# norlab-ulaval/norlab_icp_mapper

Hardware: AMD Instinct MI355X
Metric: ICP iterations/sec, 100k-pt scan vs 1M-pt map (higher is better)
Workload: dtype f32; 1 GPU; single synthetic 100000-pt scan vs 1000000-pt map, point-to-point ICP, KDTreeMatcher knn 1 maxDist 2.0 epsilon 0, TrimmedDist 0.85, fixed 20 iterations per registration; chain=p2p, scene=box+pillars sigma=0.01 seeds 42/43/44 (SURVEY.md 8d), parallelism=scan-sharded x1, map replicated

## Files before the change

norlab_icp_mapper_amd/csrc/common.h:

```cpp
#pragma once

#include <hip/hip_runtime.h>
#include <stdint.h>
#include <math.h>
#include <cstring>
#include <string>
#include <vector>
#include <unordered_map>
#include <mutex>
#include <map>
#include <cstdlib>
#include <shared_mutex>

#include "../../include/icpmi.h"

#define ICPMI_NV 32
#define ICPMI_MAX_OUTLIER 8
#define ICPMI_MAX_SMOOTH 16
#define ICPMI_SEL_BINS 2048
#ifndef ICPMI_S2_COPIES
#define ICPMI_S2_COPIES 8
#endif
#define ICPMI_S2_C0 4096
#define ICPMI_S2_F0 (ICPMI_S2_C0 + ICPMI_S2_COPIES * 256)
#ifndef ICPMI_S2_FCOPIES
#define ICPMI_S2_FCOPIES 1
#endif
#define ICPMI_S2_C1 (ICPMI_S2_F0 + ICPMI_S2_FCOPIES * 65536)
#define ICPMI_S2_F1 (ICPMI_S2_C1 + 256)
#define ICPMI_ACC_COPIES 2
#define ICPMI_ACC_MAX_ADDS 128
#define ICPMI_ACC_PAD 16
#define ICPMI_ACC_U64 (ICPMI_ACC_COPIES * ICPMI_NV * 2 * ICPMI_ACC_PAD)
#define ICPMI_ACC_IDX(copy, i, limb) ((((copy) * ICPMI_NV + (i)) * 2 + (limb)) * ICPMI_ACC_PAD)
#define ICPMI_ACC_FLAG (ICPMI_ACC_IDX(0, 0, 0) + 8)
#define ICPMI_S2_ACC (ICPMI_S2_F1 + 65536)
#define ICPMI_WIN_BINS 7
#ifndef ICPMI_WIN_COPIES
#define ICPMI_WIN_COPIES 8
#endif
#define ICPMI_WIN_PAD 16
#define ICPMI_WIN_HDR (ICPMI_WIN_COPIES * 3 * ICPMI_WIN_PAD)
#define ICPMI_WIN_U64 (ICPMI_WIN_HDR + ICPMI_WIN_PAD)
#define ICPMI_WIN_MAX_COUNT (1ll << 21)
#define ICPMI_S2_WIN (ICPMI_S2_ACC + 2 * ICPMI_ACC_U64)
#define ICPMI_SELHIST_WORDS (ICPMI_S2_WIN + 2 * ICPMI_WIN_U64)
#define ICPMI_S2_FIDX(b) ((((b) & 255u) << 8) | ((b) >> 8))

#define ICPMI_MAX_K 32

#ifdef __HIPCC__
typedef float icpmi_vf4 __attribute__((ext_vector_type(4)));
#ifdef ICPMI_NT_STREAMS
__device__ __forceinline__ float4 ld_stream(const float4* p) { const icpmi_vf4 v = __builtin_nontemporal_load(reinterpret_cast<const icpmi_vf4*>(p)); return make_float4(v.x, v.y, v.z, v.w); }
__device__ __forceinline__ float ld_stream(const float* p) { return __builtin_nontemporal_load(p); }
__device__ __forceinline__ int ld_stream(const int* p) { return __builtin_nontemporal_load(p); }
// ... 32 lines not shown
    float cell, inv_cell;
    float slack;
    int   nx, ny, nz;
    int   ncells;
};

#define ICPMI_MAXLEV 8
struct GridLevels {
    int nlev;
    GridParams g[ICPMI_MAXLEV];
    const float4* pts[ICPMI_MAXLEV];
    const unsigned* cs[ICPMI_MAXLEV];
    const unsigned* pos0[ICPMI_MAXLEV];
};

#define ICPMI_MAX_BATCH 16
struct BatchArgs {
    int nscan;
    int qstride;
    int n[ICPMI_MAX_BATCH];
};
struct BatchSrc { const float4* p[ICPMI_MAX_BATCH]; };
static inline float squared_radius(float r) { return std::isinf(r) ? INFINITY : r * r; }
static inline BatchArgs batch_of_one(int64_t n) { BatchArgs b; memset(&b, 0, sizeof b); b.nscan = 1; b.n[0] = (int)n; return b; }

struct LoopCfg {
    int   k;
    float max_dist;
    float maxr2;
    float inv1e, err2;
    int   ring_max;
    int   minimizer;
    int   n_out;
    int   out_type[ICPMI_MAX_OUTLIER];
    float out_param[ICPMI_MAX_OUTLIER];
    int   out_iparam[ICPMI_MAX_OUTLIER];
    float out_param2[ICPMI_MAX_OUTLIER];
    float out_param3[ICPMI_MAX_OUTLIER];
    int   ext;
    int   force_4dof;
    int   force_2d;
    int   is_2d;
    int   max_iter;
    int   use_diff;
    float min_rot, min_trans;
    int   smooth;
    int   use_bound;
    float max_rot, max_trans;
    int   has_read_normals;
    int   sensor_noise;
    const float* read_scalar;
};

struct IcpState {
    float T_iter[16];
    int   iter;
    int   done;
    int   error;
    int   stop_reason;
    int   counter;
    int   hist_n;
    double hq[(ICPMI_MAX_SMOOTH + 1) * 4];
    double ht[(ICPMI_MAX_SMOOTH + 1) * 3];
    double hrot[ICPMI_MAX_SMOOTH + 1];
    double htr[ICPMI_MAX_SMOOTH + 1];
    double init_q[4];
    unsigned sel_prefix;
    unsigned sel_rank;
    unsigned n_valid;
    unsigned sel_prefix_l[3];
    unsigned sel_rank_l[3];
    float limits[ICPMI_MAX_OUTLIER];
    unsigned vt_valid;
    float vt_ratio;
    float robust_med;
    float robust_scale;
    long long pairs;
    double wsum;
    unsigned hard_count;
    unsigned ticket;
    unsigned long long hard_total;
    unsigned seq;
    unsigned long long dbg[24];
    float T_prev[16];
    float T_out[16];
    unsigned long long t_start, t_done;
    unsigned long long t_nn_begin, t_nn_sum;
    unsigned nn_count, pad_nn;
};

#ifdef __HIPCC__
__device__ __forceinline__ void nn_stamp_open(IcpState* st) { st->t_nn_begin = (unsigned long long)wall_clock64(); }
__device__ __forceinline__ void nn_stamp_close(IcpState* st)
{
    const unsigned long long b = st->t_nn_begin;
    if (b) { st->t_nn_sum += (unsigned long long)wall_clock64() - b; ++st->nn_count; st->t_nn_begin = 0; }
}
#endif


inline std::shared_mutex& capture_gate() { static std::shared_mutex* m = new std::shared_mutex; return *m; }
struct CaptureGate {
    CaptureGate() { capture_gate().lock_shared(); }
    ~CaptureGate() { capture_gate().unlock_shared(); }
    CaptureGate(const CaptureGate&) = delete;
    CaptureGate& operator=(const CaptureGate&) = delete;
};

struct LoopGraph {
    hipGraphExec_t exec = nullptr; uint64_t sig = 0; int uses = 0; bool sorted = false;
    int len = 0; unsigned long used = 0;
    bool holds(uint64_t s) const { return exec && sig == s; }
    void reset() { if (exec) hipGraphExecDestroy(exec); *this = LoopGraph(); }
};
struct LoopGraphs {
    LoopGraph fixed, batch, seg[2], heads[4];
    unsigned long clock = 0;
    void reset() { fixed.reset(); batch.reset(); for (LoopGraph& g : seg) g.reset(); for (LoopGraph& g : heads) g.reset(); }
};

struct DevBlockCache {
    struct Live { size_t bytes; int dev; };
    std::mutex mu;
    std::unordered_map<void*, Live> live;
    std::map<int, std::multimap<size_t, void*>> idle_of;
    size_t idle_bytes = 0, limit = 0;
    long handles = 0;
    bool on = true;
    DevBlockCache()
    {
        const char* e = getenv("ICPMI_ALLOC_CACHE_MB");
        const long mb = e ? atol(e) : 1024;
        on = mb > 0; limit = on ? (size_t)mb << 20 : 0;
    }
};
inline DevBlockCache& dev_block_cache() { static DevBlockCache* c = new DevBlockCache; return *c; }

inline void dev_cache_release_locked(DevBlockCache& bc)
{
    for (auto& dv : bc.idle_of) for (auto& kv : dv.second) (void)hipFree(kv.second);
    bc.idle_of.clear(); bc.idle_bytes = 0;
}
inline void dev_cache_trim()
{
    DevBlockCache& bc = dev_block_cache();
    std::lock_guard<std::mutex> lk(bc.mu);
    dev_cache_release_locked(bc);
}

inline hipError_t dev_malloc(void** p, size_t bytes)
// ... 720 lines not shown
```

norlab_icp_mapper_amd/csrc/loop.hip:

```cpp
#include "common.h"
#include "solve.h"
#include <cstring>
#include <vector>

namespace {

template <int PASS, int MODE = 0>
__global__ __launch_bounds__(256) void sel_hist_kernel(const float* __restrict__ d2, int64_t count,
                                                       const IcpState* __restrict__ st, unsigned* __restrict__ ghist, int nb_scale = 0)
{
    if (st->done) return;
    if (blockIdx.x == 0 && threadIdx.x == 0) nn_stamp_close(const_cast<IcpState*>(st));
    if (MODE != 0 && nb_scale != 0 && st->iter + 1 > nb_scale) return;
    if (MODE == 3 && st->iter != 0) return;
    __shared__ unsigned h[ICPMI_SEL_BINS];
    for (int b = threadIdx.x; b < ICPMI_SEL_BINS; b += 256) h[b] = 0;
    __syncthreads();
    const unsigned prefix = st->sel_prefix;
    const float med = MODE == 2 ? st->robust_med : 0.f;
    for (int64_t i = (int64_t)blockIdx.x * 256 + threadIdx.x; i < count; i += (int64_t)gridDim.x * 256) {
        float v = d2[i];
        if (MODE == 0 || MODE == 3) { if (!(v != INFINITY && v > 0.f)) continue; }
        else {
            if (v == INFINITY) continue;
// ... 230 lines not shown
        if (win_lookup(hists, quantile, shw, pf, rr, tot)) return;
    }
#ifndef ICPMI_H0_PF
#define ICPMI_H0_PF 16
#endif
    constexpr int PF = ICPMI_H0_PF;
    const int64_t stride = (int64_t)gridDim.x * 256;
    const int64_t i0 = (int64_t)blockIdx.x * 256 + threadIdx.x;
    float pv[PF];
#pragma unroll
    for (int u = 0; u < PF; ++u) pv[u] = i0 + u * stride < count ? d2[i0 + u * stride] : INFINITY;
    if (st->done) return;
    constexpr int WIN = 4096;
    __shared__ unsigned h[256];
    __shared__ unsigned win[WIN];
    __shared__ unsigned s_top;
    h[threadIdx.x] = 0;
    for (int i = threadIdx.x; i < WIN; i += 256) win[i] = 0;
    if (threadIdx.x == 0) s_top = 0u;
    for (int64_t i = i0; i < 256 + 65536; i += stride) hists[ICPMI_S2_C1 + i] = 0;
    __syncthreads();
    {
        unsigned mx = 0;
#pragma unroll
        for (int u = 0; u < PF; ++u) if (pv[u] != INFINITY && pv[u] > 0.f) mx = max(mx, __float_as_uint(pv[u]) >> 16);
        for (int off = 32; off > 0; off >>= 1) mx = max(mx, (unsigned)__shfl_xor((int)mx, off, 64));
        if ((threadIdx.x & 63) == 0 && mx) atomicMax(&s_top, mx);
    }
    __syncthreads();
    const unsigned top = s_top + 1u, lo = top > (unsigned)WIN ? top - (unsigned)WIN : 0u;
    unsigned* fine = hists + ICPMI_S2_F0 + (blockIdx.x % ICPMI_S2_FCOPIES) * 65536;
    auto add = [&](float v) {
        if (!(v != INFINITY && v > 0.f)) return;
        const unsigned bits = __float_as_uint(v);
        const unsigned bin = bits >> 16, rel = bin - lo;
        if (rel < (unsigned)WIN) atomicAdd(&win[rel], 1u);
        else { atomicAdd(&h[bits >> 24], 1u); atomicAdd(&fine[ICPMI_S2_FIDX(bin)], 1u); }
    };
#pragma unroll
    for (int u = 0; u < PF; ++u) add(pv[u]);
    for (int64_t i = i0 + PF * stride; i < count; i += stride) add(d2[i]);
    __syncthreads();
    for (int i = threadIdx.x; i < WIN; i += 256) {
        const unsigned cnt = win[i];
        if (cnt) { const unsigned bin = lo + (unsigned)i; atomicAdd(&h[bin >> 8], cnt); atomicAdd(&fine[ICPMI_S2_FIDX(bin)], cnt); }
    }
    __syncthreads();
    if (h[threadIdx.x]) atomicAdd(&hists[ICPMI_S2_C0 + (blockIdx.x % ICPMI_S2_COPIES) * 256 + threadIdx.x], h[threadIdx.x]);
}

__global__ __launch_bounds__(256) void sel2_scan_hist_kernel(const float* __restrict__ d2, BatchArgs ba, int k, IcpState* __restrict__ st,
                                                             unsigned* __restrict__ hists, float quantile, int use_win)
{
    const int64_t count = (int64_t)ba.n[blockIdx.y] * k;
    d2 += (size_t)blockIdx.y * (size_t)ba.qstride * k;
    hists += (size_t)blockIdx.y * ICPMI_SELHIST_WORDS;
    st += blockIdx.y;
    constexpr int PF = 2;
    const int64_t stride = (int64_t)gridDim.x * 256;
    const int64_t i0 = (int64_t)blockIdx.x * 256 + threadIdx.x;
    float pv[PF];
#pragma unroll
    for (int u = 0; u < PF; ++u) pv[u] = i0 + u * stride < count ? d2[i0 + u * stride] : INFINITY;
    unsigned cv = 0;
#pragma unroll
    for (int cpy = 0; cpy < ICPMI_S2_COPIES; ++cpy) cv += hists[ICPMI_S2_C0 + cpy * 256 + threadIdx.x];
    if (st->done) return;
    if (blockIdx.x == 0 && threadIdx.x == 0) nn_stamp_close(const_cast<IcpState*>(st));
    __shared__ unsigned sh[16];
    unsigned prefix, rem, total;
    const bool win_hit = use_win && win_lookup(hists, quantile, sh, prefix, rem, total);
    if (!win_hit) block_find_rank_2tier<ICPMI_S2_FCOPIES>(cv, hists + ICPMI_S2_F0, true, quantile, 0u, sh, prefix, rem, total);
#ifndef ICPMI_NN_TIMING
    if (use_win && blockIdx.x == 0 && threadIdx.x == 0) st->dbg[win_hit ? 12 : 13] += 1ull;
#endif
    if (total == 0) {
        if (blockIdx.x == 0 && threadIdx.x == 0) { st->n_valid = 0; st->error = ICPMI_ERR_NO_OUTLIER_TO_FILTER; st->done = 1; }
        return;
    }
    if (blockIdx.x == 0 && threadIdx.x == 0) { st->sel_prefix_l[0] = prefix; st->sel_rank_l[0] = rem; st->n_valid = total; }
    auto add = [&](float v) {
        if (!(v != INFINITY && v > 0.f)) return;
        const unsigned bits = __float_as_uint(v);
        if ((bits >> 16) != prefix) return;
        atomicAdd(&hists[ICPMI_S2_C1 + ((bits >> 8) & 255u)], 1u);
        atomicAdd(&hists[ICPMI_S2_F1 + ICPMI_S2_FIDX(bits & 0xffffu)], 1u);
    };
#pragma unroll
    for (int u = 0; u < PF; ++u) add(pv[u]);
    for (int64_t i = i0 + PF * stride; i < count; i += stride) add(d2[i]);
}

constexpr int VT_CHUNK = 2048;

__global__ __launch_bounds__(256) void vt_keys_kernel(const float* __restrict__ d2, int64_t count, IcpState* __restrict__ st,
                                                      unsigned long long* __restrict__ keys, unsigned* __restrict__ vals)
{
    const int64_t i = (int64_t)blockIdx.x * 256 + threadIdx.x;
    if (blockIdx.x == 0 && threadIdx.x == 0 && !st->done) nn_stamp_close(st);
    const float v = i < count ? d2[i] : INFINITY;
    const bool valid = v != INFINITY && v > 0.f;
    if (i < count) { keys[i] = valid ? (unsigned long long)__float_as_uint(v) : 0xffffffffull; vals[i] = 0u; }
    __shared__ unsigned cnt;
    if (threadIdx.x == 0) cnt = 0;
    __syncthreads();
    const unsigned long long b = __ballot(valid);
    if ((threadIdx.x & 63) == 0 && b) atomicAdd(&cnt, (unsigned)__popcll(b));
    __syncthreads();
    if (threadIdx.x == 0 && cnt) atomicAdd(&st->vt_valid, cnt);
}

__device__ __forceinline__ double vt_value(const unsigned long long* __restrict__ sorted, int64_t i, int64_t V)
{
    return i < V ? (double)__uint_as_float((unsigned)sorted[i]) : 0.0;
}

__global__ __launch_bounds__(256) void vt_chunk_sums_kernel(const unsigned long long* __restrict__ sorted, const IcpState* __restrict__ st,
                                                            double* __restrict__ sums)
{
    const int64_t V = st->vt_valid;
    const int64_t base = (int64_t)blockIdx.x * VT_CHUNK + threadIdx.x * 8;
// ... 146 lines not shown
        else if (type == ICPMI_OUT_MINDIST) w *= (d2 >= prm * prm) ? 1.f : 0.f;
        else if (type == ICPMI_OUT_MEDIANDIST || type == ICPMI_OUT_TRIMMEDDIST || type == ICPMI_OUT_VARTRIMMEDDIST)
            w *= (d2 <= (f == fused_slot ? fused_limit : st->limits[f])) ? 1.f : 0.f;
        else if (type == ICPMI_OUT_SURFACENORMAL) {
            const float4 a = read_normals[qi];
            float ax = a.x, ay = a.y, az = a.z;
            if (T) {
                const float rx = fmaf(T[8], az, fmaf(T[4], ay, T[0] * ax));
                const float ry = fmaf(T[9], az, fmaf(T[5], ay, T[1] * ax));
                const float rz = fmaf(T[10], az, fmaf(T[6], ay, T[2] * ax));
                ax = rx; ay = ry; az = rz;
            }
            const float4 b = ref_normals[sidx];
            const float dot = fmaf(az, b.z, fmaf(ay, b.y, ax * b.x));
            w *= (dot > cosf(prm)) ? 1.f : 0.f;
        } else if (EXT && type == ICPMI_OUT_GENERICDESCRIPTOR) {
            const int ip = lc.out_iparam[f];
            const float v = (ip & ICPMI_GEN_SOURCE_READING) ? lc.read_scalar[qi] : ref_scalar[orig];
            w *= (ip & ICPMI_GEN_SOFT) ? v : ((ip & ICPMI_GEN_LARGER) ? (v > prm ? 1.f : 0.f) : (v < prm ? 1.f : 0.f));
        } else if (EXT && type == ICPMI_OUT_ROBUST) {
            const int ip = lc.out_iparam[f];
            const int se = (ip >> 4) & 15, fct = ip & 15;
            const float sc = se != ICPMI_SCALE_NONE ? st->robust_scale : 1.f;
            const float res = ((ip >> 8) & 15) == ICPMI_DIST_POINT2PLANE ? plane2 : d2;
            const float kk = se != ICPMI_SCALE_BERG ? prm : (fct == ICPMI_ROB_CAUCHY ? 4.3040f : fct == ICPMI_ROB_TUKEY ? 7.0589f : fct == ICPMI_ROB_HUBER ? 2.0138f : prm);
            const float e2 = res / (sc * sc);
            const float apx = lc.out_param3[f];
            float rw = robust_weight(fct, e2, kk);
            if (apx > 0.f && apx != INFINITY && e2 >= apx * apx) rw = 0.f;
            w *= rw;
        }
    }
    return w;
}

__host__ __device__ __forceinline__ int acc_threads(int k) { return k > 1 ? 1024 : 256; }
__host__ __device__ __forceinline__ int acc_blocks_dev(int64_t count, int cap, int bt = 256)
{
    const int64_t nb = (count + bt - 1) / bt;
    return (int)(nb < 1 ? 1 : (nb > cap ? cap : nb));
}

template <int MIN, bool FUSED, bool EXT, int BT = 256>
__global__ __launch_bounds__(BT) void accumulate_kernel(const float4* __restrict__ reading, BatchArgs ba, int acc_cap, LoopCfg lc,
                                                         IcpState* __restrict__ st, const float4* __restrict__ map,
                                                         const float4* __restrict__ normals,
                                                         const float4* __restrict__ read_normals,
                                                         const int* __restrict__ sidx, const float* __restrict__ d2a,
                                                         unsigned* __restrict__ hists,
                                                         int fused_slot, int is_median, float factor,
                                                         const float4* __restrict__ match_pt, const int* __restrict__ qindex,
                                                         const float* __restrict__ ref_scalar, const float4* __restrict__ pnm)
{
    const int n = ba.n[blockIdx.y];
    const int nbe = acc_blocks_dev((int64_t)n * lc.k, acc_cap, BT);
    if ((int)blockIdx.x >= nbe) return;
    {
        const size_t qo = (size_t)blockIdx.y * (size_t)ba.qstride;
        reading += qo; sidx += qo * lc.k; d2a += qo * lc.k;
        if (match_pt) match_pt += qo;
        if (qindex) qindex += qo;
        if (read_normals) read_normals += qo;
        hists += (size_t)blockIdx.y * ICPMI_SELHIST_WORDS;
        st += blockIdx.y;
    }
    const int64_t count = (int64_t)n * lc.k;
    const int64_t stride = (int64_t)nbe * BT;
    const int64_t gtid = (int64_t)blockIdx.x * BT + threadIdx.x;
#ifdef ICPMI_ACC_STRIDED
    const int64_t estep = stride;
    const int64_t e_first = gtid, e_end = count;
#else
    const int64_t estep = BT;
    const int wgc = (nbe & 7) == 0 ? (int)(blockIdx.x & 7) * (nbe >> 3) + (int)(blockIdx.x >> 3) : (int)blockIdx.x;
    const int64_t per_wg = (count + nbe - 1) / nbe;
    const int64_t e_first = (int64_t)wgc * per_wg + threadIdx.x;
    const int64_t e_end = ((int64_t)wgc + 1) * per_wg < count ? ((int64_t)wgc + 1) * per_wg : count;
#endif
    constexpr int PF = BT > 256 ? 3 : 2;
    float pd2[PF]; int ps[PF]; float4 pr[PF], pq[PF];
#pragma unroll
    for (int u = 0; u < PF; ++u) {
        const int64_t e = e_first + u * estep;
        const bool in = e < e_end;
        pd2[u] = in ? ld_stream(d2a + e) : INFINITY;
        ps[u] = in ? ld_stream(sidx + e) : -1;
        pr[u] = ld_stream(reading + (in ? (int)(e / lc.k) : 0));
        pq[u] = (match_pt && in) ? ld_stream(match_pt + e) : ((pnm && ps[u] >= 0) ? pnm[2 * (size_t)ps[u]] : make_float4(0.f, 0.f, 0.f, 0.f));
    }
    const unsigned cv = (FUSED && threadIdx.x < 256) ? hists[ICPMI_S2_C1 + threadIdx.x] : 0u;
    float4 pn[PF];
#pragma unroll
    for (int u = 0; u < PF; ++u)
        pn[u] = (MIN == ICPMI_MIN_POINT_TO_PLANE && ps[u] >= 0) ? (pnm ? pnm[2 * (size_t)ps[u] + 1] : normals[ps[u]]) : make_float4(0.f, 0.f, 0.f, 0.f);
    if (st->done) return;
    if (blockIdx.x == 0 && threadIdx.x == 0) nn_stamp_close(const_cast<IcpState*>(st));
    float fused_limit = 0.f;
    if (FUSED) {
        __shared__ unsigned shsel[16];
        unsigned bin, rem, total;
        block_find_rank_2tier<1>(cv, hists + ICPMI_S2_F1, false, 0.f, st->sel_rank_l[0], shsel, bin, rem, total);
        const float q = __uint_as_float((st->sel_prefix_l[0] << 16) | bin);
        fused_limit = is_median ? factor * q : q;
        if (blockIdx.x == 0 && threadIdx.x == 0) st->limits[fused_slot] = fused_limit;
        for (int64_t i = gtid; i < ICPMI_S2_COPIES * 256 + ICPMI_S2_FCOPIES * 65536; i += stride) hists[ICPMI_S2_C0 + i] = 0;
        if (lc.k > 1) for (int64_t i = gtid; i < 2 * ICPMI_WIN_U64; i += stride) hists[ICPMI_S2_WIN + i] = 0;
    }
    constexpr int NVAL = MIN == ICPMI_MIN_POINT_TO_PLANE ? 27 : (MIN == ICPMI_MIN_POINT_TO_POINT ? 16 : 0);
    double acc[NVAL > 0 ? NVAL : 1];
#pragma unroll
    for (int i = 0; i < (NVAL > 0 ? NVAL : 1); ++i) acc[i] = 0.0;
    double wsum = 0.0, cnt = 0.0;
    double b2d[3] = {0.0, 0.0, 0.0};
    const float* T = st->T_iter;
    auto pair = [&](int64_t e, float d2, int s, float4 r, float4 qkept, float4 nkept, bool have_n) {
        if (d2 == INFINITY) return;
        const int qi = (int)(e / lc.k);
        float w;
        if (EXT) {
            const float3 pe = xf_point(T, r.x, r.y, r.z, r.w);
            const float4 qe = (match_pt || (pnm && have_n)) ? qkept : (pnm ? pnm[2 * (size_t)s] : map[s]);
            float plane2 = 0.f;
            if (normals) {
                const float4 ne = have_n && MIN == ICPMI_MIN_POINT_TO_PLANE ? nkept : (pnm ? pnm[2 * (size_t)s + 1] : normals[s]);
                const float dx = pe.x - qe.x, dy = pe.y - qe.y, dz = pe.z - qe.z;
                const float dot = dx * ne.x + dy * ne.y + dz * ne.z;
                plane2 = dot * dot;
            }
            w = match_weight<true>(lc, st, d2, T, read_normals, qindex ? qindex[qi] : qi, normals, s, FUSED ? fused_slot : -1, fused_limit,
                                   ref_scalar, __float_as_int(qe.w), plane2);
        } else w = match_weight(lc, st, d2, T, read_normals, qindex ? qindex[qi] : qi, normals, s, FUSED ? fused_slot : -1, fused_limit);
        if (w == 0.f) return;
        wsum += w; cnt += 1.0;
        if (MIN == ICPMI_MIN_IDENTITY) return;
        const float3 p = xf_point(T, r.x, r.y, r.z, r.w);
        const float4 q = (match_pt || (pnm && have_n)) ? qkept : (pnm ? pnm[2 * (size_t)s] : map[s]);
        if (MIN == ICPMI_MIN_POINT_TO_POINT) {
            const double dw = w;
            acc[0] += dw;
            acc[1] += dw * p.x; acc[2] += dw * p.y; acc[3] += dw * p.z;
            acc[4] += dw * q.x; acc[5] += dw * q.y; acc[6] += dw * q.z;
            const double wq[3] = {dw * q.x, dw * q.y, dw * q.z};
            const float pc[3] = {p.x, p.y, p.z};
#pragma unroll
            for (int c = 0; c < 3; ++c)
#pragma unroll
                for (int rr = 0; rr < 3; ++rr) acc[7 + 3 * c + rr] += wq[rr] * pc[c];
        } else if (MIN == ICPMI_MIN_POINT_TO_PLANE) {
            const float4 nn = have_n ? nkept : (pnm ? pnm[2 * (size_t)s + 1] : normals[s]);
            const float F[6] = {p.y * nn.z - p.z * nn.y, p.z * nn.x - p.x * nn.z, p.x * nn.y - p.y * nn.x, nn.x, nn.y, nn.z};
            const float dx = p.x - q.x, dy = p.y - q.y, dz = p.z - q.z;
            const float dot = dx * nn.x + dy * nn.y + dz * nn.z;
            int idx = 0;
#pragma unroll
            for (int a = 0; a < 6; ++a) {
                const double wf = (double)w * F[a];
#pragma unroll
                for (int b = a; b < 6; ++b) acc[idx++] += wf * F[b];
                acc[21 + a] -= wf * dot;
            }
            if (EXT && lc.force_2d) {
                const float dot2 = dx * nn.x + dy * nn.y;
#pragma unroll
                for (int a = 0; a < 3; ++a) b2d[a] -= ((double)w * F[2 + a]) * dot2;
            }
        }
    };
// ... 605 lines not shown
                               nn.built_win ? 1 : 0);
        }
        int hb2 = (int)std::min<int64_t>((count + 511) / 512, 512);
        if (hb2 < 1) hb2 = 1;
        hipLaunchKernelGGL(sel2_scan_hist_kernel, dim3(hb2, ba.nscan), dim3(256), 0, c->stream, c->d_d2, ba, lc.k, c->d_state, c->d_selhist, quant,
                           (nn.built_win && !nn.built_hist0) ? 1 : 0);
        return;
    }
    for (int f = 0; f < lc.n_out; ++f) {
        const int type = lc.out_type[f];
        if (type != ICPMI_OUT_TRIMMEDDIST && type != ICPMI_OUT_MEDIANDIST) continue;
        const int is_med = type == ICPMI_OUT_MEDIANDIST;
        const float quant = is_med ? 0.5f : lc.out_param[f];
        const float factor = lc.out_param[f];
        hipLaunchKernelGGL((sel_hist_kernel<0, 0>), dim3(hb), dim3(256), 0, c->stream, c->d_d2, count, c->d_state, c->d_selhist, 0);
        hipLaunchKernelGGL(sel_scan_kernel<0>, dim3(1), dim3(256), 0, c->stream, c->d_state, c->d_selhist, quant, f, is_med, factor, 0, 0);
        hipLaunchKernelGGL((sel_hist_kernel<1, 0>), dim3(hb), dim3(256), 0, c->stream, c->d_d2, count, c->d_state, c->d_selhist, 0);
        hipLaunchKernelGGL(sel_scan_kernel<1>, dim3(1), dim3(256), 0, c->stream, c->d_state, c->d_selhist, quant, f, is_med, factor, 0, 0);
        hipLaunchKernelGGL((sel_hist_kernel<2, 0>), dim3(hb), dim3(256), 0, c->stream, c->d_d2, count, c->d_state, c->d_selhist, 0);
        hipLaunchKernelGGL(sel_scan_kernel<2>, dim3(1), dim3(256), 0, c->stream, c->d_state, c->d_selhist, quant, f, is_med, factor, 0, 0);
    }
}

template <int MIN, bool FUSED, bool EXT>
static void launch_accumulate_ext(icpmi_ctx* c, const LoopCfg& lc, int nb, int slot, const BatchArgs& ba, bool sorted);

template <int MIN, bool FUSED>
static void launch_accumulate(icpmi_ctx* c, const LoopCfg& lc, int nb, int slot, const BatchArgs& ba, bool sorted)
{
    if (lc.ext) launch_accumulate_ext<MIN, FUSED, true>(c, lc, nb, slot, ba, sorted);
    else launch_accumulate_ext<MIN, FUSED, false>(c, lc, nb, slot, ba, sorted);
}

template <int MIN, bool FUSED, bool EXT>
static void launch_accumulate_ext(icpmi_ctx* c, const LoopCfg& lc, int nb, int slot, const BatchArgs& ba, bool sorted)
{
    const float4* rn = lc.has_read_normals ? c->d_read_normals : nullptr;
    const int is_med = slot >= 0 && lc.out_type[slot] == ICPMI_OUT_MEDIANDIST;
    const float factor = slot >= 0 ? lc.out_param[slot] : 0.f;
    if (lc.k > 1) {
        hipLaunchKernelGGL((accumulate_kernel<MIN, FUSED, EXT, 1024>), dim3(nb, ba.nscan), dim3(1024), 0, c->stream, sorted ? c->d_qsorted : c->d_reading, ba, acc_cap(), lc, c->d_state,
                           c->d_map_sorted, c->has_normals ? c->d_normals_sorted : (const float4*)nullptr, rn, c->d_sidx, c->d_d2, c->d_selhist, slot, is_med, factor,
                           (const float4*)nullptr, sorted ? c->d_qindex : (const int*)nullptr, (EXT && c->raw_has_scalar) ? c->d_raw_s : (const float*)nullptr,
                           (MIN == ICPMI_MIN_POINT_TO_PLANE && c->has_normals && c->d_map_pn) ? c->d_map_pn : (const float4*)nullptr);
        return;
    }
    hipLaunchKernelGGL((accumulate_kernel<MIN, FUSED, EXT>), dim3(nb, ba.nscan), dim3(256), 0, c->stream, sorted ? c->d_qsorted : c->d_reading, ba, acc_cap(), lc, c->d_state,
                       c->d_map_sorted, c->has_normals ? c->d_normals_sorted : (const float4*)nullptr, rn, c->d_sidx, c->d_d2, c->d_selhist, slot, is_med, factor,
                       (sorted && lc.k == 1) ? c->d_match_pt : (const float4*)nullptr, sorted ? c->d_qindex : (const int*)nullptr,
                       (EXT && c->raw_has_scalar) ? c->d_raw_s : (const float*)nullptr,
                       (lc.k > 1 && MIN == ICPMI_MIN_POINT_TO_PLANE && c->has_normals && c->d_map_pn) ? c->d_map_pn : (const float4*)nullptr);
}

static void enqueue_accumulate_solve(icpmi_ctx* c, int64_t n, const LoopCfg& lc, const BatchArgs& ba, const NnOutcome& nn, float* d_Tstep, double* d_sums)
{
    const int64_t count = n * lc.k;
    const int nb = acc_blocks(count, acc_threads(lc.k));
    const int slot = fused_filter_slot(lc);
    const bool fused = slot >= 0;
    if (lc.minimizer == ICPMI_MIN_POINT_TO_PLANE) {
        if (fused) launch_accumulate<ICPMI_MIN_POINT_TO_PLANE, true>(c, lc, nb, slot, ba, nn.out_sorted);
        else launch_accumulate<ICPMI_MIN_POINT_TO_PLANE, false>(c, lc, nb, slot, ba, nn.out_sorted);
    } else if (lc.minimizer == ICPMI_MIN_POINT_TO_POINT) {
        if (fused) launch_accumulate<ICPMI_MIN_POINT_TO_POINT, true>(c, lc, nb, slot, ba, nn.out_sorted);
        else launch_accumulate<ICPMI_MIN_POINT_TO_POINT, false>(c, lc, nb, slot, ba, nn.out_sorted);
    } else {
        if (fused) launch_accumulate<ICPMI_MIN_IDENTITY, true>(c, lc, nb, slot, ba, nn.out_sorted);
        else launch_accumulate<ICPMI_MIN_IDENTITY, false>(c, lc, nb, slot, ba, nn.out_sorted);
    }
    hipLaunchKernelGGL(solve_kernel, dim3(ba.nscan), dim3(256), 0, c->stream, c->d_state, c->d_selhist, 1, lc, d_Tstep, d_sums,
                       c->d_progress, ba.nscan == 1 ? c->d_state_mirror : (IcpState*)nullptr);
}

static NnRequest loop_request(icpmi_ctx* c, const LoopCfg& lc, const BatchArgs& ba, const float* d_r2row)
{
    NnRequest req;
    req.hist0 = fused_filter_slot(lc) >= 0 ? c->d_selhist.get() : nullptr;
    req.match_pt = lc.k == 1 ? c->d_match_pt.get() : nullptr;
    req.sorted_k = lc.k > 1;
    req.r2row = d_r2row;
    req.batch = ba;
    return req;
}

static icpmi_status enqueue_iteration(icpmi_ctx* c, int64_t n, const LoopCfg& lc, const NnRequest& req, NnOutcome* nn, hipEvent_t nn0, hipEvent_t nn1)
{
    if (nn0) HIP_TRY(c, hipEventRecord(nn0, c->stream));
    icpmi_status s = nn_launch_k(c, req, c->d_reading, n, c->d_state->T_iter, lc, 1, c->d_sidx, c->d_d2, c->d_state, nn);
    if (s != ICPMI_OK) return s;
    if (nn1) HIP_TRY(c, hipEventRecord(nn1, c->stream));
    enqueue_selection(c, lc, n * lc.k, req.batch, *nn);
    enqueue_accumulate_solve(c, n, lc, req.batch, *nn, nullptr, req.batch.nscan > 1 ? nullptr : c->d_keep_sums.get());
    HIP_TRY(c, hipGetLastError());
    return ICPMI_OK;
}

static void fill_stats(const IcpState* hs, const LoopCfg& lc, int64_t n, icpmi_stats* stats, bool with_dbg = true)
{
    if (!stats) return;
    stats->iterations = hs->iter;
    stats->stop_reason = hs->stop_reason;
    stats->pairs = hs->pairs;
    const double denom = (double)lc.k * (double)n;
    stats->point_used_ratio = denom > 0 ? (float)hs->pairs / (float)denom : 0.f;
    stats->weighted_point_used_ratio = denom > 0 ? (float)(hs->wsum / denom) : 0.f;
    stats->trimmed_limit = -1.f;
    for (int f = 0; f < lc.n_out; ++f)
        if (lc.out_type[f] == ICPMI_OUT_TRIMMEDDIST || lc.out_type[f] == ICPMI_OUT_MEDIANDIST || lc.out_type[f] == ICPMI_OUT_VARTRIMMEDDIST) stats->trimmed_limit = hs->limits[f];
    stats->hard_queries = (int64_t)hs->hard_total;
    stats->sensor_noise_overlap = -1.f;
    for (int i = 0; i < 2 && with_dbg; ++i) { stats->reserved[2 * i] = (int32_t)(hs->dbg[i] & 0xffffffffu); stats->reserved[2 * i + 1] = (int32_t)(hs->dbg[i] >> 32); }
}

static void host_mat4_mul(const float* A, const float* B, float* C)
{
    float R[16];
    for (int j = 0; j < 4; ++j)
        for (int i = 0; i < 4; ++i) {
            float s = A[i] * B[4 * j];
            for (int kk = 1; kk < 4; ++kk) s = fmaf(A[4 * kk + i], B[4 * j + kk], s);
            R[4 * j + i] = s;
        }
    memcpy(C, R, sizeof R);
}

static void pose_out(const icpmi_ctx* c, const float* T_iter, float* T_out)
{
    float Tm[16], Tmi[16], tmp[16];
    for (int i = 0; i < 16; ++i) Tm[i] = Tmi[i] = (i % 5 == 0) ? 1.f : 0.f;
    for (int r = 0; r < 3; ++r) { Tm[12 + r] = c->mean[r]; Tmi[12 + r] = -c->mean[r]; }
    host_mat4_mul(T_iter, Tmi, tmp);
    host_mat4_mul(Tm, tmp, T_out);
}

static icpmi_status enqueue_registration_head(icpmi_ctx* c, const float4* d_scan, const float* d_normals3, int64_t n)
{
    bool head_done = false;
    icpmi_status s = loop_prepare_reading(c, d_scan, n, d_normals3, &head_done);
    if (s != ICPMI_OK) return s;
    if (head_done) return ICPMI_OK;
    hipLaunchKernelGGL(init_state_kernel, dim3(1), dim3(64), 0, c->stream, c->d_state, (const float*)nullptr, c->reg_seq, c->d_progress,
                       (const unsigned*)(c->d_progress + 32));
    HIP_TRY(c, hipMemsetAsync(c->d_selhist, 0, ICPMI_SELHIST_WORDS * sizeof(unsigned), c->stream));
    HIP_TRY(c, hipGetLastError());
    return ICPMI_OK;
// ... 15 lines not shown
    hipGraphDestroy(gr);
    HIP_TRY(c, ie);
    g.sig = sig; g.uses = 1; g.sorted = nn.out_sorted;
    return ICPMI_OK;
}

static uint64_t loop_sig(const icpmi_ctx* c, const LoopCfg& lc, const NnRequest& req, const float4* d_scan, const float* d_normals3, int64_t n)
{
    uint64_t sig = fnv(&lc, sizeof lc, 1469598103934665603ull);
    const void* ptrs[] = {d_scan, d_normals3, c->d_qkeys, c->d_qtile, c->d_reading, c->d_read_normals, c->d_sidx, c->d_d2, c->d_hard, c->d_state, c->d_match_pt,
                          c->d_qsorted, c->d_qindex, c->d_map_sorted, c->d_normals_sorted, c->d_cell_start, c->d_selhist, req.r2row,
                          c->scratch[0], c->scratch[1], c->scratch[2], c->scratch[3], c->scratch[4]};
    sig = fnv(ptrs, sizeof ptrs, sig);
    sig = fnv(&c->grid, sizeof c->grid, sig);
    sig = fnv(&c->map_epoch, sizeof c->map_epoch, sig);
    return fnv(&n, sizeof n, sig);
}

static bool go_eager(icpmi_ctx* c, int* wasted, bool cached, uint64_t sig)
{
    if (cached || *wasted < 2) return false;
    if (c->eager_sig == sig) { *wasted = 0; return false; }
    c->eager_sig = sig;
    return true;
}

icpmi_status loop_run(icpmi_ctx* c, const float4* d_scan, const float* d_normals3, int64_t n, const LoopCfg& lc_in, const float* d_r2row,
                      bool fixed, float T_out[16], icpmi_stats* stats)
{
    LoopCfg lc = lc_in;
    c->last_match_n = 0; c->cov_ready = false; c->cov_kept = false;
    if (ensure_loop_buffers(c, n, lc.k) != ICPMI_OK) return ICPMI_ERR_HIP;
    if (chain_has_vartrimmed(lc)) { VtBuffers vb; if (vt_buffers(c, n * lc.k, &vb) != ICPMI_OK) return ICPMI_ERR_HIP; }
    if (c->d_reading.ensure(c, (size_t)n + 1) != ICPMI_OK) return ICPMI_ERR_HIP;
    if (d_normals3 && c->d_read_normals.ensure(c, (size_t)n + 1) != ICPMI_OK) return ICPMI_ERR_HIP;
    if (c->cfg.knn <= 8 && sort_queries_reserve(c, n) != ICPMI_OK) return ICPMI_ERR_HIP;
    NnRequest req = loop_request(c, lc, batch_of_one(n), d_r2row);
    NnOutcome last;

    const bool profile = c->cfg.profile != 0;
    bool graph = c->cfg.use_graph != 0 && fixed && !profile;
    float nn_ms_sum = 0.f; int nn_cnt = 0;
    c->reg_seq = (c->reg_seq + 1) & 0x7ffffu;
    __atomic_store_n(c->h_progress + 32, c->reg_seq, __ATOMIC_RELEASE);
    const bool fast_ok = !profile && c->d_state_mirror && lc.max_iter < 0xfff;
    if (!fast_ok) HIP_TRY(c, hipEventRecord(c->ev0, c->stream));
    bool segmented = !graph && !profile && c->cfg.use_graph != 0 && (lc.use_diff || lc.use_bound) && lc.max_iter < 0xfff && lc.max_iter > 1;
    const int S = std::min(4, lc.max_iter);
    LoopGraphs& gs = c->graphs;
    const uint64_t sig = (graph || segmented) ? loop_sig(c, lc, req, d_scan, d_normals3, n) : 0;
    const bool cached = segmented ? gs.seg[0].holds(sig) && gs.seg[1].holds(sig) : gs.fixed.holds(sig);
    if (segmented && go_eager(c, &c->seg_wasted, cached, sig)) segmented = false;
    if (graph && go_eager(c, &c->graph_wasted, cached, sig)) graph = false;
    auto enqueue_loop = [&](bool with_head, int first, int count, NnOutcome* nn) {
        icpmi_status s = with_head ? enqueue_registration_head(c, d_scan, d_normals3, n) : ICPMI_OK;
        for (int it = 0; it < count && s == ICPMI_OK; ++it) { req.iter = first + it; s = enqueue_iteration(c, n, lc, req, nn, nullptr, nullptr); }
        return s;
    };
    if (!graph && !segmented) {
        icpmi_status s = enqueue_registration_head(c, d_scan, d_normals3, n);
        if (s != ICPMI_OK) return s;
    }
    if (segmented) {
        ++gs.seg[0].uses;
        if (!cached) {
            for (LoopGraph& hd : gs.heads) hd.reset();
            for (int g = 0; g < 2; ++g) {
                const icpmi_status s = capture_loop_graph(c, gs.seg[g], sig, [&](NnOutcome* nn) { return enqueue_loop(g == 0, g == 0 ? 0 : S, S, nn); });
                if (s != ICPMI_OK) return s;
            }
        }
        LoopGraph* head = &gs.seg[0];
        const int L = c->seg_prev_iters;
        if (L >= 2 && L != S && L <= 24 && L < lc.max_iter) {
            head = nullptr;
            for (LoopGraph& hd : gs.heads) if (hd.exec && hd.len == L) head = &hd;
            if (!head) {
                head = &gs.heads[0];
                for (LoopGraph& hd : gs.heads) if (!hd.exec) { head = &hd; break; } else if (hd.used < head->used) head = &hd;
                const icpmi_status s = capture_loop_graph(c, *head, sig, [&](NnOutcome* nn) { return enqueue_loop(true, 0, L, nn); });
                if (s != ICPMI_OK) return s;
                head->len = L;
            }
            head->used = ++gs.clock;
        }
        const int head_len = head == &gs.seg[0] ? S : L;
        HIP_TRY(c, hipGraphLaunch(head->exec, c->stream));
        if (c->cfg.knn <= 8) { c->qsorted_n = n; c->qsorted_src = c->d_reading; }
        int launched = head_len;
        while (launched < lc.max_iter) {
            const int lead = (launched == head_len && head_len != S) ? 0 : (S > 1 ? S / 2 : 1);
            unsigned v = 0; bool idle = false;
            HIP_TRY(c, spin_on_host(c->stream, 256, c->h_progress, 1, &v, [&](const unsigned* w) {
                const ProgressWord p = decode_progress(*w, c->reg_seq);
                return p.mine && (p.done || p.iter + lead >= launched);
            }, &idle));
            const ProgressWord p = decode_progress(v, c->reg_seq);
            if (idle ? !p.mine || p.done || p.iter < launched : p.done) break;
            HIP_TRY(c, hipGraphLaunch(gs.seg[1].exec, c->stream));
            launched += S;
        }
    } else if (graph) {
        ++gs.fixed.uses;
        if (!cached) {
            const icpmi_status s = capture_loop_graph(c, gs.fixed, sig, [&](NnOutcome* nn) { return enqueue_loop(true, 0, lc.max_iter, nn); });
            if (s != ICPMI_OK) return s;
        }
        HIP_TRY(c, hipGraphLaunch(gs.fixed.exec, c->stream));
        if (c->cfg.knn <= 8) { c->qsorted_n = n; c->qsorted_src = c->d_reading; }
    } else {
        const int check_every = (lc.use_diff || lc.use_bound) ? 4 : lc.max_iter;
        if (profile && c->nn_events.size() < (size_t)2 * lc.max_iter) {
            while (c->nn_events.size() < (size_t)2 * lc.max_iter) {
                hipEvent_t e; HIP_TRY(c, hipEventCreate(&e)); c->nn_events.push_back(e);
            }
        }
        constexpr int ahead = 2;
        const bool poll = !profile && (lc.use_diff || lc.use_bound) && lc.max_iter < 0xfff;
        int launched = 0;
        bool stopped = false;
        for (int it = 0; it < lc.max_iter && !stopped; ++it) {
            hipEvent_t e0 = profile ? c->nn_events[2 * it] : nullptr, e1 = profile ? c->nn_events[2 * it + 1] : nullptr;
            req.iter = it;
            icpmi_status s = enqueue_iteration(c, n, lc, req, &last, e0, e1);
            if (s != ICPMI_OK) return s;
            ++launched;
            if (it + 1 >= lc.max_iter) break;
            if (poll) {
                unsigned v = 0; bool idle = false;
                HIP_TRY(c, spin_on_host(c->stream, 256, c->h_progress, 1, &v, [&](const unsigned* w) {
                    const ProgressWord p = decode_progress(*w, c->reg_seq);
                    return p.mine && (p.done || p.iter + ahead > it);
                }, &idle));
                const ProgressWord p = decode_progress(v, c->reg_seq);
                stopped = idle ? !p.mine || p.done || p.iter <= it : p.done;
            } else if ((it + 1) % check_every == 0) {
                const IcpState* sd = c->d_state;
                HIP_TRY(c, hipMemcpyAsync(&c->h_state->done, &sd->done, sizeof(int), hipMemcpyDeviceToHost, c->stream));
                HIP_TRY(c, hipStreamSynchronize(c->stream));
                if (c->h_state->done) break;
            }
        }
        if (profile) {
            if (c->nn_events.size() < (size_t)2 * lc.max_iter + 2) {
                while (c->nn_events.size() < (size_t)2 * lc.max_iter + 2) { hipEvent_t e; HIP_TRY(c, hipEventCreate(&e)); c->nn_events.push_back(e); }
            }
            HIP_TRY(c, hipEventRecord(c->nn_events[2 * lc.max_iter], c->stream));
            HIP_TRY(c, hipEventRecord(c->nn_events[2 * lc.max_iter + 1], c->stream));
            HIP_TRY(c, hipStreamSynchronize(c->stream));
            HIP_TRY(c, hipMemcpy(c->h_state, c->d_state, sizeof(IcpState), hipMemcpyDeviceToHost));
            const int iters_done = c->h_state->iter < launched ? c->h_state->iter : launched;
            for (int it = 0; it < iters_done; ++it) {
                float ms = 0.f;
                if (hipEventElapsedTime(&ms, c->nn_events[2 * it], c->nn_events[2 * it + 1]) == hipSuccess) { nn_ms_sum += ms; ++nn_cnt; }
            }
            float gap = 0.f;
            if (hipEventElapsedTime(&gap, c->nn_events[2 * lc.max_iter], c->nn_events[2 * lc.max_iter + 1]) == hipSuccess && nn_cnt) {
                nn_ms_sum -= gap * nn_cnt;
// ... 530 lines not shown
```

Baseline: 23870 iterations/s.

## Pack hot ICP state into a wave-wide header and skip intermediate progress publishes

Moves the per-iteration fields the kernels read (T_iter, done, selection prefix and rank, t_nn_begin and others) into a 256-byte aligned header at the start of IcpState. Each wave loads it with one coalesced dword-per-lane read and pulls fields out with readlane, replacing scattered scalar loads that sat on the critical path of the selection and accumulate kernels. The NN timing stamp now uses atomics. In the fixed-graph path only the last iteration's solve publishes the progress word, which removes per-iteration host-visible writes. The struct reorder touches every user of IcpState, and empty asm barriers are added to pin values in scalar and vector registers.

```diff
diff --git a/norlab_icp_mapper_amd/csrc/common.h b/norlab_icp_mapper_amd/csrc/common.h
--- a/norlab_icp_mapper_amd/csrc/common.h
+++ b/norlab_icp_mapper_amd/csrc/common.h
@@ -2,6 +2,7 @@
 
 #include <hip/hip_runtime.h>
 #include <stdint.h>
+#include <stddef.h>
 #include <math.h>
 #include <cstring>
 #include <string>
@@ -140,14 +141,28 @@
     const float* read_scalar;
 };
 
-struct IcpState {
+struct alignas(128) LoopHdr {
     float T_iter[16];
     int   iter;
     int   done;
     int   error;
-    int   stop_reason;
     int   counter;
     int   hist_n;
+    unsigned seq;
+    unsigned hard_count;
+    unsigned n_valid;
+    unsigned sel_prefix_l[3];
+    unsigned sel_rank_l[3];
+    float robust_scale;
+    unsigned pad_hdr;
+    float limits[ICPMI_MAX_OUTLIER];
+    unsigned long long t_nn_begin;
+};
+static_assert(sizeof(LoopHdr) == 256 && alignof(LoopHdr) == 128, "the loop header is two 128-byte lines: one dword per lane of a wave");
+#define ICPMI_HDR_W(field) ((int)(offsetof(LoopHdr, field) / 4))
+
+struct IcpState : LoopHdr {
+    int   stop_reason;
     double hq[(ICPMI_MAX_SMOOTH + 1) * 4];
     double ht[(ICPMI_MAX_SMOOTH + 1) * 3];
     double hrot[ICPMI_MAX_SMOOTH + 1];
@@ -155,35 +170,40 @@
     double init_q[4];
     unsigned sel_prefix;
     unsigned sel_rank;
-    unsigned n_valid;
-    unsigned sel_prefix_l[3];
-    unsigned sel_rank_l[3];
-    float limits[ICPMI_MAX_OUTLIER];
     unsigned vt_valid;
     float vt_ratio;
     float robust_med;
-    float robust_scale;
     long long pairs;
     double wsum;
-    unsigned hard_count;
     unsigned ticket;
     unsigned long long hard_total;
-    unsigned seq;
     unsigned long long dbg[24];
     float T_prev[16];
     float T_out[16];
     unsigned long long t_start, t_done;
-    unsigned long long t_nn_begin, t_nn_sum;
+    unsigned long long t_nn_sum;
     unsigned nn_count, pad_nn;
 };
 
 #ifdef __HIPCC__
+__device__ __forceinline__ unsigned hdr_load(const IcpState* st) { return reinterpret_cast<const unsigned*>(st)[threadIdx.x & 63]; }
+struct HdrView {
+    unsigned w;
+    __device__ __forceinline__ unsigned u(int i) const { return (unsigned)__builtin_amdgcn_readlane((int)w, i); }
+    __device__ __forceinline__ int i(int idx) const { return __builtin_amdgcn_readlane((int)w, idx); }
+    __device__ __forceinline__ float f(int idx) const { return __int_as_float(__builtin_amdgcn_readlane((int)w, idx)); }
+    __device__ __forceinline__ unsigned long long u64(int idx) const { return (unsigned long long)u(idx) | ((unsigned long long)u(idx + 1) << 32); }
+};
 __device__ __forceinline__ void nn_stamp_open(IcpState* st) { st->t_nn_begin = (unsigned long long)wall_clock64(); }
-__device__ __forceinline__ void nn_stamp_close(IcpState* st)
-{
-    const unsigned long long b = st->t_nn_begin;
-    if (b) { st->t_nn_sum += (unsigned long long)wall_clock64() - b; ++st->nn_count; st->t_nn_begin = 0; }
-}
+__device__ __forceinline__ void nn_stamp_close(IcpState* st, unsigned long long b)
+{
+    if (b) {
+        atomicAdd(&st->t_nn_sum, (unsigned long long)wall_clock64() - b);
+        atomicAdd(&st->nn_count, 1u);
+        st->t_nn_begin = 0;
+    }
+}
+__device__ __forceinline__ void nn_stamp_close(IcpState* st) { nn_stamp_close(st, st->t_nn_begin); }
 #endif
 
 
diff --git a/norlab_icp_mapper_amd/csrc/loop.hip b/norlab_icp_mapper_amd/csrc/loop.hip
--- a/norlab_icp_mapper_amd/csrc/loop.hip
+++ b/norlab_icp_mapper_amd/csrc/loop.hip
@@ -306,6 +306,7 @@
 __global__ __launch_bounds__(256) void sel2_scan_hist_kernel(const float* __restrict__ d2, BatchArgs ba, int k, IcpState* __restrict__ st,
                                                              unsigned* __restrict__ hists, float quantile, int use_win)
 {
+    asm volatile("" ::"s"(ba.n[blockIdx.y]), "s"(ba.qstride), "s"(k), "s"(d2), "s"(hists), "s"(st), "s"(quantile), "s"(use_win));
     const int64_t count = (int64_t)ba.n[blockIdx.y] * k;
     d2 += (size_t)blockIdx.y * (size_t)ba.qstride * k;
     hists += (size_t)blockIdx.y * ICPMI_SELHIST_WORDS;
@@ -313,14 +314,16 @@
     constexpr int PF = 2;
     const int64_t stride = (int64_t)gridDim.x * 256;
     const int64_t i0 = (int64_t)blockIdx.x * 256 + threadIdx.x;
+    HdrView hv{hdr_load(st)};
     float pv[PF];
 #pragma unroll
     for (int u = 0; u < PF; ++u) pv[u] = i0 + u * stride < count ? d2[i0 + u * stride] : INFINITY;
     unsigned cv = 0;
 #pragma unroll
     for (int cpy = 0; cpy < ICPMI_S2_COPIES; ++cpy) cv += hists[ICPMI_S2_C0 + cpy * 256 + threadIdx.x];
-    if (st->done) return;
-    if (blockIdx.x == 0 && threadIdx.x == 0) nn_stamp_close(const_cast<IcpState*>(st));
+    asm volatile("" : "+v"(hv.w), "+v"(pv[0]), "+v"(pv[1]), "+v"(cv));
+    if (hv.i(ICPMI_HDR_W(done))) return;
+    if (blockIdx.x == 0 && threadIdx.x == 0) nn_stamp_close(st, hv.u64(ICPMI_HDR_W(t_nn_begin)));
     __shared__ unsigned sh[16];
     unsigned prefix, rem, total;
     const bool win_hit = use_win && win_lookup(hists, quantile, sh, prefix, rem, total);
@@ -573,6 +576,9 @@
                                                          const float4* __restrict__ match_pt, const int* __restrict__ qindex,
                                                          const float* __restrict__ ref_scalar, const float4* __restrict__ pnm)
 {
+    asm volatile("" ::"s"(ba.n[blockIdx.y]), "s"(ba.qstride), "s"(acc_cap), "s"(lc.k), "s"(lc.n_out), "s"(lc.out_type[0]), "s"(lc.out_param[0]),
+                 "s"(reading), "s"(sidx), "s"(d2a), "s"(match_pt), "s"(qindex), "s"(read_normals), "s"(hists), "s"(st), "s"(map), "s"(normals),
+                 "s"(pnm), "s"(fused_slot), "s"(is_median), "s"(factor));
     const int n = ba.n[blockIdx.y];
     const int nbe = acc_blocks_dev((int64_t)n * lc.k, acc_cap, BT);
     if ((int)blockIdx.x >= nbe) return;
@@ -599,6 +605,7 @@
     const int64_t e_end = ((int64_t)wgc + 1) * per_wg < count ? ((int64_t)wgc + 1) * per_wg : count;
 #endif
     constexpr int PF = BT > 256 ? 3 : 2;
+    unsigned hw = hdr_load(st);
     float pd2[PF]; int ps[PF]; float4 pr[PF], pq[PF];
 #pragma unroll
     for (int u = 0; u < PF; ++u) {
@@ -609,19 +616,27 @@
         pr[u] = ld_stream(reading + (in ? (int)(e / lc.k) : 0));
         pq[u] = (match_pt && in) ? ld_stream(match_pt + e) : ((pnm && ps[u] >= 0) ? pnm[2 * (size_t)ps[u]] : make_float4(0.f, 0.f, 0.f, 0.f));
     }
-    const unsigned cv = (FUSED && threadIdx.x < 256) ? hists[ICPMI_S2_C1 + threadIdx.x] : 0u;
+    unsigned cv = (FUSED && threadIdx.x < 256) ? hists[ICPMI_S2_C1 + threadIdx.x] : 0u;
+    asm volatile("" : "+v"(hw), "+v"(cv));
+    const HdrView hv{hw};
+    const int done = hv.i(ICPMI_HDR_W(done));
+    const unsigned long long t_nn_begin = hv.u64(ICPMI_HDR_W(t_nn_begin));
+    const unsigned sel_rank0 = hv.u(ICPMI_HDR_W(sel_rank_l)), sel_prefix0 = hv.u(ICPMI_HDR_W(sel_prefix_l));
+    float T[16];
+#pragma unroll
+    for (int i = 0; i < 16; ++i) T[i] = hv.f(ICPMI_HDR_W(T_iter) + i);
     float4 pn[PF];
 #pragma unroll
     for (int u = 0; u < PF; ++u)
         pn[u] = (MIN == ICPMI_MIN_POINT_TO_PLANE && ps[u] >= 0) ? (pnm ? pnm[2 * (size_t)ps[u] + 1] : normals[ps[u]]) : make_float4(0.f, 0.f, 0.f, 0.f);
-    if (st->done) return;
-    if (blockIdx.x == 0 && threadIdx.x == 0) nn_stamp_close(const_cast<IcpState*>(st));
+    if (done) return;
+    if (blockIdx.x == 0 && threadIdx.x == 0) nn_stamp_close(st, t_nn_begin);
     float fused_limit = 0.f;
     if (FUSED) {
         __shared__ unsigned shsel[16];
         unsigned bin, rem, total;
-        block_find_rank_2tier<1>(cv, hists + ICPMI_S2_F1, false, 0.f, st->sel_rank_l[0], shsel, bin, rem, total);
-        const float q = __uint_as_float((st->sel_prefix_l[0] << 16) | bin);
+        block_find_rank_2tier<1>(cv, hists + ICPMI_S2_F1, false, 0.f, sel_rank0, shsel, bin, rem, total);
+        const float q = __uint_as_float((sel_prefix0 << 16) | bin);
         fused_limit = is_median ? factor * q : q;
         if (blockIdx.x == 0 && threadIdx.x == 0) st->limits[fused_slot] = fused_limit;
         for (int64_t i = gtid; i < ICPMI_S2_COPIES * 256 + ICPMI_S2_FCOPIES * 65536; i += stride) hists[ICPMI_S2_C0 + i] = 0;
@@ -633,7 +648,6 @@
     for (int i = 0; i < (NVAL > 0 ? NVAL : 1); ++i) acc[i] = 0.0;
     double wsum = 0.0, cnt = 0.0;
     double b2d[3] = {0.0, 0.0, 0.0};
-    const float* T = st->T_iter;
     auto pair = [&](int64_t e, float d2, int s, float4 r, float4 qkept, float4 nkept, bool have_n) {
         if (d2 == INFINITY) return;
         const int qi = (int)(e / lc.k);
@@ -1345,7 +1359,8 @@
                        (lc.k > 1 && MIN == ICPMI_MIN_POINT_TO_PLANE && c->has_normals && c->d_map_pn) ? c->d_map_pn : (const float4*)nullptr);
 }
 
-static void enqueue_accumulate_solve(icpmi_ctx* c, int64_t n, const LoopCfg& lc, const BatchArgs& ba, const NnOutcome& nn, float* d_Tstep, double* d_sums)
+static void enqueue_accumulate_solve(icpmi_ctx* c, int64_t n, const LoopCfg& lc, const BatchArgs& ba, const NnOutcome& nn, float* d_Tstep, double* d_sums,
+                                     bool publish = true)
 {
     const int64_t count = n * lc.k;
     const int nb = acc_blocks(count, acc_threads(lc.k));
@@ -1362,7 +1377,7 @@
         else launch_accumulate<ICPMI_MIN_IDENTITY, false>(c, lc, nb, slot, ba, nn.out_sorted);
     }
     hipLaunchKernelGGL(solve_kernel, dim3(ba.nscan), dim3(256), 0, c->stream, c->d_state, c->d_selhist, 1, lc, d_Tstep, d_sums,
-                       c->d_progress, ba.nscan == 1 ? c->d_state_mirror : (IcpState*)nullptr);
+                       publish ? c->d_progress : (unsigned*)nullptr, ba.nscan == 1 ? c->d_state_mirror : (IcpState*)nullptr);
 }
 
 static NnRequest loop_request(icpmi_ctx* c, const LoopCfg& lc, const BatchArgs& ba, const float* d_r2row)
@@ -1376,14 +1391,15 @@
     return req;
 }
 
-static icpmi_status enqueue_iteration(icpmi_ctx* c, int64_t n, const LoopCfg& lc, const NnRequest& req, NnOutcome* nn, hipEvent_t nn0, hipEvent_t nn1)
+static icpmi_status enqueue_iteration(icpmi_ctx* c, int64_t n, const LoopCfg& lc, const NnRequest& req, NnOutcome* nn, hipEvent_t nn0, hipEvent_t nn1,
+                                      bool publish = true)
 {
     if (nn0) HIP_TRY(c, hipEventRecord(nn0, c->stream));
     icpmi_status s = nn_launch_k(c, req, c->d_reading, n, c->d_state->T_iter, lc, 1, c->d_sidx, c->d_d2, c->d_state, nn);
     if (s != ICPMI_OK) return s;
     if (nn1) HIP_TRY(c, hipEventRecord(nn1, c->stream));
     enqueue_selection(c, lc, n * lc.k, req.batch, *nn);
-    enqueue_accumulate_solve(c, n, lc, req.batch, *nn, nullptr, req.batch.nscan > 1 ? nullptr : c->d_keep_sums.get());
+    enqueue_accumulate_solve(c, n, lc, req.batch, *nn, nullptr, req.batch.nscan > 1 ? nullptr : c->d_keep_sums.get(), publish);
     HIP_TRY(c, hipGetLastError());
     return ICPMI_OK;
 }
@@ -1505,9 +1521,12 @@
     const bool cached = segmented ? gs.seg[0].holds(sig) && gs.seg[1].holds(sig) : gs.fixed.holds(sig);
     if (segmented && go_eager(c, &c->seg_wasted, cached, sig)) segmented = false;
     if (graph && go_eager(c, &c->graph_wasted, cached, sig)) graph = false;
-    auto enqueue_loop = [&](bool with_head, int first, int count, NnOutcome* nn) {
+    auto enqueue_loop = [&](bool with_head, int first, int count, NnOutcome* nn, bool last_word_only = false) {
         icpmi_status s = with_head ? enqueue_registration_head(c, d_scan, d_normals3, n) : ICPMI_OK;
-        for (int it = 0; it < count && s == ICPMI_OK; ++it) { req.iter = first + it; s = enqueue_iteration(c, n, lc, req, nn, nullptr, nullptr); }
+        for (int it = 0; it < count && s == ICPMI_OK; ++it) {
+            req.iter = first + it;
+            s = enqueue_iteration(c, n, lc, req, nn, nullptr, nullptr, !last_word_only || it + 1 == count);
+        }
         return s;
     };
     if (!graph && !segmented) {
@@ -1556,7 +1575,7 @@
     } else if (graph) {
         ++gs.fixed.uses;
         if (!cached) {
-            const icpmi_status s = capture_loop_graph(c, gs.fixed, sig, [&](NnOutcome* nn) { return enqueue_loop(true, 0, lc.max_iter, nn); });
+            const icpmi_status s = capture_loop_graph(c, gs.fixed, sig, [&](NnOutcome* nn) { return enqueue_loop(true, 0, lc.max_iter, nn, true); });
             if (s != ICPMI_OK) return s;
         }
         HIP_TRY(c, hipGraphLaunch(gs.fixed.exec, c->stream));
```

Result: faster. 24460 iterations/s, median of 6 (+2.5%).
